# damlobster/DotsBoxesAZ

Hardware: AMD Instinct MI355X
Metric: mcts_node_expansions_per_sec (higher is better)
Workload: dtype f32 via f16x3 (hi,lo)-split MFMA, f32 accumulate; max |dp|,|dv| vs torch fp32 = 1e-6 (tests/test_hip_nn.py)

## Files before the change

dotsboxesaz_amd/build.py:

```python
import hashlib
import os
import subprocess
import sys
from concurrent.futures import ThreadPoolExecutor

HERE = os.path.dirname(os.path.abspath(__file__))
CSRC = os.path.join(HERE, "csrc")
LIB = os.path.join(HERE, "libdbaz_hip.so")
HIPCC = os.environ.get("HIPCC", "/opt/rocm/bin/hipcc")
ARCH = "gfx950"

UNITS = [
    ("tree.hip", ["-ffp-contract=off"]),
    ("engine.hip", []),
    ("nn.hip", []),
    ("replay.hip", ["-ffp-contract=off"]),
    ("train.hip", []),
    ("train_net.hip", []),
]
COMMON = ["--offload-arch=" + ARCH, "-O3", "-fPIC", "-std=c++17", "-Wall", "-Wno-unused-function"]


def source_files():
    fs = [os.path.join(CSRC, f) for f in sorted(os.listdir(CSRC)) if f.endswith((".hip", ".h"))]
    return fs + [os.path.join(os.path.dirname(HERE), "include", "dbaz.h")]


def source_hash(only=None):
    h = hashlib.sha256()
    for f in source_files():
        if only is not None and os.path.basename(f) not in only:
            continue
        h.update(os.path.basename(f).encode() + b"\0")
        h.update(open(f, "rb").read())
    return h.hexdigest()[:16]


NN_SOURCES = ("nn.hip", "nn.h", "common.h")


def _newer(target, deps):
    if not os.path.exists(target):
        return True
    t = os.path.getmtime(target)
    return any(os.path.getmtime(d) > t for d in deps)


def build(force=False, verbose=False):
    hdrs = [os.path.join(CSRC, f) for f in os.listdir(CSRC) if f.endswith(".h")]
    hdrs.append(os.path.join(os.path.dirname(HERE), "include", "dbaz.h"))
    objs, jobs = [], []
    for src, extra in UNITS:
        s = os.path.join(CSRC, src)
        o = os.path.join(CSRC, src.replace(".hip", ".o"))
        objs.append(o)
        if force or _newer(o, [s] + hdrs):
            jobs.append([HIPCC] + COMMON + extra + ["-c", s, "-o", o])

    def run(cmd):
        if verbose:
            print(" ".join(cmd), flush=True)
        r = subprocess.run(cmd, stdout=subprocess.PIPE, stderr=subprocess.STDOUT, text=True)
        if r.returncode != 0:
            raise RuntimeError("hipcc failed:\n%s\n%s" % (" ".join(cmd), r.stdout))
        return r.stdout

    sh = source_hash() + " nn=" + source_hash(NN_SOURCES)
    bo, bh = os.path.join(CSRC, "buildinfo.o"), os.path.join(CSRC, "buildinfo.hash")
    objs.append(bo)
    if force or not os.path.exists(bo) or not os.path.exists(bh) or open(bh).read() != sh:
        jobs.append(["g++", "-O1", "-fPIC", "-c", os.path.join(CSRC, "buildinfo.cpp"), "-o", bo, '-DDBAZ_SRC_HASH="%s"' % sh])

    with ThreadPoolExecutor(max_workers=4) as ex:
        outs = list(ex.map(run, jobs))
    open(bh, "w").write(sh)
    if verbose:
        for o in outs:
            if o.strip():
                print(o)
    if jobs or force or _newer(LIB, objs):
        run([HIPCC, "--offload-arch=" + ARCH, "-shared", "-fPIC", "-o", LIB] + objs)
    return LIB


if __name__ == "__main__":
    print(build(force="--force" in sys.argv, verbose=True))
```

dotsboxesaz_amd/csrc/nn.hip:

```cpp
#include <math.h>
#include <stddef.h>
#include <stdlib.h>
#include <string.h>

#include <map>
#include <string>
#include <vector>

#include "nn.h"

typedef float f32x4 __attribute__((ext_vector_type(4)));

#define CONV_THREADS 512
#define MAXT 13
#define MAXROWS 256

struct NNState {
    Geo g;
    int max_batch = 0, precision = 0;
    int kind = 0, C = 0 , Craw = 0 , blocks = 0, hc = 0, vf = 0;
    bool ready = false;
    std::map<std::string, std::vector<float>> sd;
    std::vector<float> osc_host;
    std::vector<void *> allocs;
    float *in_s = nullptr, *in_t = nullptr;
    float *w0 = nullptr, *b0 = nullptr;
    float *tw = nullptr, *tb = nullptr;
    float *tosc = nullptr;
    unsigned long long *stamp_out = nullptr;
    int *overflow = nullptr;
    int *ovf_flags = nullptr;
    float *tw32 = nullptr, *tb32 = nullptr;
    float *hw = nullptr, *hb = nullptr;
    float *w0p = nullptr;
    float osc0 = 1.0f;
    float *hwp = nullptr;
    float hosc = 1.0f;
    float *wfc = nullptr, *bfc = nullptr;
    int KP = 0, ntp = 0, ntv = 0;
    float *wv1 = nullptr, *bv1 = nullptr;
    float *hact = nullptr;
    size_t fc_lds = 0;
    float *sn_s0 = nullptr, *sn_t0 = nullptr, *sn_ts = nullptr, *sn_tt = nullptr;
    float *sn_flat = nullptr, *sn_h1 = nullptr;
    float *sn_w0 = nullptr, *sn_b0 = nullptr, *sn_ps0 = nullptr, *sn_pt0 = nullptr;
    float *sn_w1 = nullptr, *sn_b1 = nullptr, *sn_ps1 = nullptr, *sn_pt1 = nullptr;
    size_t sn_lds = 0;
    int S = 1, NT = 1, NTT = 7;
    int S_small = 0, S_mid = 0, S_big = 0, cus = 256;
    size_t conv_lds = 0;
    int c2 = 0, S_c2 = 0, NT_c2 = 0;
    int use_rem = 0;
    size_t conv_lds_c2 = 0;
};

template <int C, int NTT>
__device__ __forceinline__ void conv_lds_f32(const f32x4 *__restrict__ src4, f32x4 *dst4, const float *__restrict__ wpk,
                                             const float *__restrict__ bias, const int *vm, int rowbase, int zbase,
                                             int W, int R, int wave, int lane, int residual, int tbase,
                                             const float *post_s = nullptr, const float *post_t = nullptr)
{
    constexpr int S4 = (C + 8) / 4;
    constexpr int KC = C / 16;
    const int jrow = lane & 15, gq = lane >> 4;
    for (int ct = wave & 3; ct < C / 16; ct += 4) {
        f32x4 acc[NTT];
#pragma unroll
        for (int t = 0; t < NTT; t++) acc[t] = (f32x4){0.f, 0.f, 0.f, 0.f};
        const f32x4 *wbase = reinterpret_cast<const f32x4 *>(wpk) + (size_t)ct * 9 * KC * 64 + lane;
        int addr[NTT];
#pragma unroll
        for (int t = 0; t < NTT; t++) addr[t] = (vm[t] & 1) ? rowbase + (-W - 1) * S4 : zbase + ((rowbase + (-W - 1) * S4) & 15) - t * 16 * S4;
        f32x4 a_cur = wbase[0];
        f32x4 b_cur[NTT];
#pragma unroll
        for (int t = 0; t < NTT; t++) b_cur[t] = src4[addr[t] + t * 16 * S4];
#pragma unroll 1
        for (int tap = 0; tap < 9; tap++) {
#pragma unroll
            for (int kc = 0; kc < KC; kc++) {
                f32x4 a_nxt, b_nxt[NTT];
                if (kc == KC - 1) {
                    const int tn = tap + 1;
                    const int off = ((tn / 3 - 1) * W + (tn % 3 - 1)) * S4;
#pragma unroll
                    for (int t = 0; t < NTT; t++) addr[t] = ((vm[t] >> tn) & 1) ? rowbase + off : zbase + ((rowbase + off) & 15) - t * 16 * S4;
                    a_nxt = wbase[(size_t)(tn < 9 ? tn * KC : 0) * 64];
#pragma unroll
                    for (int t = 0; t < NTT; t++) b_nxt[t] = src4[addr[t] + t * 16 * S4];
                } else {
// ... 211 lines not shown
            }
        }
        float vmax = 0.0f;
#pragma unroll
        for (int t = 0; t < NTT; t++) {
            const int row = (tbase + t) * 16 + jrow;
            f32x4 v = acc[t] * oscale + bv;
            if (residual) {
                if constexpr (RR) {
                    v += res[t];
                } else {
                    union { unsigned int u; f16x2 h; } c0, c1, d0, d1;
                    c0.u = rh[t][0]; c1.u = rh[t][1]; d0.u = rl[t][0]; d1.u = rl[t][1];
                    v[0] += (float)c0.h[0] + (float)d0.h[0];
                    v[1] += (float)c0.h[1] + (float)d0.h[1];
                    v[2] += (float)c1.h[0] + (float)d1.h[0];
                    v[3] += (float)c1.h[1] + (float)d1.h[1];
                }
            }
            v = relu4(v);
            if constexpr (RR) {
                if (residual) res[t] = v;
            }
            if (post_s) {
                v = v * *reinterpret_cast<const f32x4 *>(post_s + ct * 16 + gq * 4) +
                    *reinterpret_cast<const f32x4 *>(post_t + ct * 16 + gq * 4);
                vmax = fmaxf(vmax, fmaxf(fmaxf(fabsf(v[0]), fabsf(v[1])), fmaxf(fabsf(v[2]), fabsf(v[3]))));
            } else {
                vmax = fmaxf(vmax, max4(v));
            }
            h3_store<C>(dsth + (size_t)row * (S4 * 8) + ct * 16 + gq * 4, row < R, v);
        }
        ovf |= vmax > F16_GUARD;
        STAMP(t3);
#ifdef DBAZ_STAMP
        if (stamps) { stamps[0] += t1 - t0; stamps[1] += t2 - t1; stamps[2] += t3 - t2; }
#endif
    }
    ovf_out |= ovf;
}

#define WRING_UNITS 512

__device__ __forceinline__ void glds16(const void *gsrc, unsigned lds_dst)
{
    unsigned keep;
    asm volatile("s_mov_b32 %0, m0\n\ts_mov_b32 m0, %2\n\ts_nop 0\n\tglobal_load_lds_dwordx4 %1, off\n\ts_mov_b32 m0, %0"
                 : "=&s"(keep) : "v"(gsrc), "s"(lds_dst) : "memory");
}
__device__ __forceinline__ unsigned lds_addr(const void *p)
{
    return (unsigned)(size_t)(const __attribute__((address_space(3))) char *)p;
}
template <int C, int NTT>
__device__ __forceinline__ void conv_lds_h3_c2(const f32x4 *__restrict__ src4, f32x4 *dst4, const f32x4 *__restrict__ wpk ,
                                               const float *__restrict__ bias, float oscale, const int *vm, int rowbase,
                                               int zbase, int W, int R, int wave, int lane, int residual, bool &ovf_out, int tbase,
                                               WPre (&pre)[2], const f32x4 *next_wpk, f32x4 (&res)[2][NTT],
                                               unsigned long long *stamps, f32x4 *wring)
{
    unsigned long long t0 = 0, t1 = 0, t2 = 0, t3 = 0;
    (void)t0; (void)t1; (void)t2; (void)t3; (void)stamps;
    static_assert(C == 64, "two cout tiles per wave x two wave parities = 64 channels");
    constexpr int S4 = (C + 8) / 4;
    constexpr int KS = C / 32;
    constexpr int LO = C / 8;
    constexpr int N = 9 * KS;
    static_assert(N % 2 == 0, "the next layer's step 0 must land in slot 0");
    const int jrow = lane & 15, gq = lane >> 4;
    const int ct0 = (wave & 1) * 2;
    f32x4 acc[2][NTT];
#pragma unroll
    for (int c = 0; c < 2; c++)
#pragma unroll
        for (int t = 0; t < NTT; t++) acc[c][t] = (f32x4){0.f, 0.f, 0.f, 0.f};
    u128h a_h[2][2], a_l[2][2];
    u128h bh[NTT], bl[NTT];
    const char *sb = reinterpret_cast<const char *>(src4);
    int ab[NTT];
    auto tap_unit = [&](int offr) -> int { return rowbase + offr * S4; };
    {
        const int u0 = tap_unit(-W - 1);
#pragma unroll
        for (int t = 0; t < NTT; t++) ab[t] = ((vm[t] & 1) ? u0 : zbase + (u0 & 15) - t * 16 * S4) * 16;
    }
    STAMP(t0);
    const f32x4 *dsrc = wpk + ((size_t)(wave >> 1) * N * 2 + (wave & 1)) * 64 + lane;
    const f32x4 *dnext = next_wpk ? next_wpk + ((size_t)(wave >> 1) * N * 2 + (wave & 1)) * 64 + lane : nullptr;
    const f32x4 *rsrc = wring + (size_t)ct0 * 2 * 64 + lane;
    const unsigned ring_dst = __builtin_amdgcn_readfirstlane(lds_addr(wring + (size_t)wave * 64));
#pragma unroll
    for (int c = 0; c < 2; c++) { a_h[c][0].f = pre[c].h0; a_l[c][0].f = pre[c].l0; }
#pragma unroll
    for (int t = 0; t < NTT; t++) bh[t].f = *reinterpret_cast<const f32x4 *>(sb + ab[t] + t * 256 * S4);
#pragma unroll
    for (int t = 0; t < NTT; t++) bl[t].f = *reinterpret_cast<const f32x4 *>(sb + ab[t] + t * 256 * S4 + LO * 16);
    STAMP(t1);
#pragma unroll
    for (int i = 0; i < N; i++) {
        const int cur = i & 1, nxt = (i + 1) & 1;
        const int ni = i + 1, ntap = ni / KS, nks = ni % KS;
        if (i + 2 < N) glds16(dsrc + (size_t)(i + 2) * 128, ring_dst + (i & 1) * (WRING_UNITS * 16));
        else if (dnext) glds16(dnext + (size_t)(i + 2 - N) * 128, ring_dst + (i & 1) * (WRING_UNITS * 16));
        if (ni < N) {
            const f32x4 *r1 = rsrc + (size_t)(ni & 1) * WRING_UNITS;
            a_h[0][nxt].f = r1[0]; a_l[0][nxt].f = r1[64]; a_h[1][nxt].f = r1[128]; a_l[1][nxt].f = r1[192];
        }
        __builtin_amdgcn_sched_barrier(0);
#pragma unroll
        for (int t = 0; t < NTT; t++) {
            acc[0][t] = __builtin_amdgcn_mfma_f32_16x16x32_f16(a_h[0][cur].h, bh[t].h, acc[0][t], 0, 0, 0);
            acc[1][t] = __builtin_amdgcn_mfma_f32_16x16x32_f16(a_h[1][cur].h, bh[t].h, acc[1][t], 0, 0, 0);
        }
        if (ni < N && nks == 0) {
            const int un = tap_unit((ntap / 3 - 1) * W + (ntap % 3 - 1));
            const int zt = zbase + (un & 15);
#pragma unroll
            for (int t = 0; t < NTT; t++) ab[t] = (((vm[t] >> ntap) & 1) ? un : zt - t * 16 * S4) * 16;
        }
        __builtin_amdgcn_sched_barrier(0);
#pragma unroll
        for (int t = 0; t < NTT; t++) {
            acc[0][t] = __builtin_amdgcn_mfma_f32_16x16x32_f16(a_l[0][cur].h, bh[t].h, acc[0][t], 0, 0, 0);
            acc[1][t] = __builtin_amdgcn_mfma_f32_16x16x32_f16(a_l[1][cur].h, bh[t].h, acc[1][t], 0, 0, 0);
            if (ni < N) bh[t].f = *reinterpret_cast<const f32x4 *>(sb + ab[t] + t * 256 * S4 + nks * 64);
            __builtin_amdgcn_sched_barrier(0);
        }
#pragma unroll
        for (int t = 0; t < NTT; t++) {
            acc[0][t] = __builtin_amdgcn_mfma_f32_16x16x32_f16(a_h[0][cur].h, bl[t].h, acc[0][t], 0, 0, 0);
            acc[1][t] = __builtin_amdgcn_mfma_f32_16x16x32_f16(a_h[1][cur].h, bl[t].h, acc[1][t], 0, 0, 0);
            if (ni < N) bl[t].f = *reinterpret_cast<const f32x4 *>(sb + ab[t] + t * 256 * S4 + nks * 64 + LO * 16);
            __builtin_amdgcn_sched_barrier(0);
        }
        if (ni < N) asm volatile("s_waitcnt vmcnt(0) lgkmcnt(%0)" ::"n"(2 * NTT) : "memory");
        else asm volatile("s_waitcnt vmcnt(0)" ::: "memory");
        if (ni < N) __builtin_amdgcn_s_barrier();
        __builtin_amdgcn_sched_barrier(0);
    }
    STAMP(t2);
    f32x4 bv[2];
#pragma unroll
    for (int c = 0; c < 2; c++) {
        bv[c] = *reinterpret_cast<const f32x4 *>(bias + (ct0 + c) * 16 + gq * 4);
        asm volatile("" ::"v"(bv[c]));
    }
    __builtin_amdgcn_sched_barrier(0);
    if (next_wpk) {
        pre[0].h0 = rsrc[0]; pre[0].l0 = rsrc[64]; pre[1].h0 = rsrc[128]; pre[1].l0 = rsrc[192];
    }
    __builtin_amdgcn_sched_barrier(0);
    _Float16 *dsth = reinterpret_cast<_Float16 *>(dst4);
    float vmax = 0.0f;
#pragma unroll
    for (int c = 0; c < 2; c++) {
        const int col = (ct0 + c) * 16 + gq * 4;
#pragma unroll
        for (int t = 0; t < NTT; t++) {
            const int row = (tbase + t) * 16 + jrow;
            f32x4 v = acc[c][t] * oscale + bv[c];
            if (residual) v += res[c][t];
            v = relu4(v);
            if (residual) res[c][t] = v;
            vmax = fmaxf(vmax, max4(v));
            h3_store<C>(dsth + (size_t)row * (S4 * 8) + col, row < R, v);
        }
    }
    ovf_out |= vmax > F16_GUARD;
    STAMP(t3);
#ifdef DBAZ_STAMP
    if (stamps) { stamps[0] += t1 - t0; stamps[1] += t2 - t1; stamps[2] += t3 - t2; }
#endif
}

__device__ __forceinline__ int cut_n(int n, int round, int defer_max)
{
    if (round <= 0) return n;
    const int n_full = (n / round) * round;
    return (n_full > 0 && n - n_full <= defer_max) ? n_full : n;
}

struct TowerArgs {
    const float *feat;
    const int32_t *list;
    const int32_t *n_dev;
    const float *in_s, *in_t;
    const float *w0, *b0;
    const float *tw;
    const float *tb;
    const float *tosc;
    const float *hw, *hb;
    const float *hwp;
    float hosc;
    const float *w0p;
    float osc0;
    unsigned long long *stamp_out;
    const float *wfc, *bfc;
    const float *wv1, *bv1;
    float *P, *V;
    int KP, ntp, ntv, vf, AS;
    int32_t *n_used;
    int *overflow;
    int *ovf_flags;
    int fallback;
    int S, nblocks, hc;
    int role, S_main, S_small, S_mid, S_big, S_huge, cus;
    int cut_round, cut_defer;
};
static_assert(offsetof(TowerArgs, wfc) == 136, "see stamp_out: the fields from wfc on keep these kernel-argument offsets");

__device__ __forceinline__ void head_fc_fused(const Geo &g, const TowerArgs &a, const float *stage, float *lg, int ns, int s0,
                                              int tid, int nthr)
{
    const int lane = tid & 63, wave = tid >> 6, nw = nthr >> 6;
    const int K = a.hc * g.HW, KC = a.KP / 16, NJ = a.ntp + a.ntv, LGS = NJ * 16 + 1, A = g.A;
    const int jrow = lane & 15, gq = lane >> 4;
    const f32x4 *wfc4 = reinterpret_cast<const f32x4 *>(a.wfc);
    const float *rowp = stage + (size_t)min(jrow, ns - 1) * (2 * K) + gq * 4;
    constexpr int G = 8;
    for (int job = wave; job < NJ; job += nw) {
        const float *brow = rowp + (job < a.ntp ? 0 : K);
        const f32x4 *wp = wfc4 + (size_t)job * KC * 64 + lane;
        f32x4 acc = (f32x4){0.f, 0.f, 0.f, 0.f};
        f32x4 wc[G], wn[G];
#pragma unroll
        for (int j = 0; j < G; j++) wc[j] = j < KC ? wp[(size_t)j * 64] : (f32x4){0.f, 0.f, 0.f, 0.f};
        for (int base = 0; base < KC; base += G) {
#pragma unroll
            for (int j = 0; j < G; j++) wn[j] = base + G + j < KC ? wp[(size_t)(base + G + j) * 64] : (f32x4){0.f, 0.f, 0.f, 0.f};
#pragma unroll
            for (int j = 0; j < G; j++)
                if (base + j < KC) {
                    const f32x4 b = *reinterpret_cast<const f32x4 *>(brow + (base + j) * 16);
#pragma unroll
                    for (int e = 0; e < 4; e++) acc = __builtin_amdgcn_mfma_f32_16x16x4f32(wc[j][e], b[e], acc, 0, 0, 0);
                }
#pragma unroll
            for (int j = 0; j < G; j++) wc[j] = wn[j];
        }
        if (jrow < ns) {
#pragma unroll
            for (int e = 0; e < 4; e++) lg[jrow * LGS + job * 16 + gq * 4 + e] = acc[e] + a.bfc[job * 16 + gq * 4 + e];
        }
    }
    __syncthreads();
    for (int sidx = wave; sidx < ns; sidx += nw) {
        const int dst = a.list ? a.list[s0 + sidx] : s0 + sidx;
        const float *l = lg + sidx * LGS;
        float mx = -INFINITY;
        for (int o = lane; o < A; o += 64) mx = fmaxf(mx, l[o]);
        for (int sh = 32; sh > 0; sh >>= 1) mx = fmaxf(mx, __shfl_xor(mx, sh));
        float sum = 0.0f;
        for (int o = lane; o < A; o += 64) sum += expf(l[o] - mx);
        for (int sh = 32; sh > 0; sh >>= 1) sum += __shfl_xor(sum, sh);
        for (int o = lane; o < A; o += 64) a.P[(size_t)dst * a.AS + o] = expf(l[o] - mx) / sum;
        float hv = 0.0f;
        for (int u = lane; u < a.vf; u += 64) hv += fmaxf(l[a.ntp * 16 + u], 0.0f) * a.wv1[u];
        for (int sh = 32; sh > 0; sh >>= 1) hv += __shfl_xor(hv, sh);
        if (lane == 0) a.V[dst] = tanhf(hv + a.bv1[0]);
    }
// ... 85 lines not shown
                    al.f = wp[64];
                    const f32x4 bv = *reinterpret_cast<const f32x4 *>(a.b0 + cto * 16 + gg * 4) * ACT_SCALE;
                    _Float16 *dsth = reinterpret_cast<_Float16 *>(X4);
                    float vmax = 0.0f;
                    for (int t = half; t < NT; t += nhalf) {
                        const int row = t * 16 + jr;
                        const int rr = min(row, R - 1);
                        u128h bh, bl;
                        bh.f = M4[(size_t)rr * MU + gg];
                        bl.f = M4[(size_t)rr * MU + 4 + gg];
                        f32x4 acc = (f32x4){0.f, 0.f, 0.f, 0.f};
                        acc = __builtin_amdgcn_mfma_f32_16x16x32_f16(ah.h, bh.h, acc, 0, 0, 0);
                        acc = __builtin_amdgcn_mfma_f32_16x16x32_f16(al.h, bh.h, acc, 0, 0, 0);
                        acc = __builtin_amdgcn_mfma_f32_16x16x32_f16(ah.h, bl.h, acc, 0, 0, 0);
                        f32x4 v = acc * a.osc0 + bv;
                        v = relu4(v);
                        vmax = fmaxf(vmax, max4(v));
                        h3_store<C>(dsth + (size_t)row * (S4 * 8) + cto * 16 + gg * 4, row < R, v);
                    }
                    ovf |= vmax > F16_GUARD;
                }
            }
        }
        if (!mfma0) {
        for (int i = tid; i < R * (C / 16); i += NTHR) {
            const int row = i % R, cq = i / R;
            const float *pp = pad + rowbase_s[row];
            float in27[27];
#pragma unroll
            for (int tap = 0; tap < 9; tap++)
#pragma unroll
                for (int c = 0; c < 3; c++) in27[tap * 3 + c] = pp[(c * PH + tap / 3) * PW + tap % 3];
#pragma unroll
            for (int q = 0; q < 4; q++) {
                const int co = cq * 16 + q * 4;
                f32x4 acc = *reinterpret_cast<const f32x4 *>(a.b0 + co);
#pragma unroll
                for (int k = 0; k < 27; k++) acc += in27[k] * *reinterpret_cast<const f32x4 *>(wl + k * C + co);
#pragma unroll
                for (int e = 0; e < 4; e++) act_store<C, PREC>(X, row, co + e, fmaxf(acc[e], 0.0f), ovf);
            }
        }
        }
        __syncthreads();
        if (tid < 3 * S4) {
            X4[zu + tid] = (f32x4){0.f, 0.f, 0.f, 0.f};
            Y4[zu + tid] = (f32x4){0.f, 0.f, 0.f, 0.f};
        }
    }
    __syncthreads();
    const int jrow = lane & 15, gq = lane >> 4;
    const bool first = wave < 4;
    const int tbase = C2 ? (wave >> 1) * NTA : (first ? 0 : NTA);
    int vm[NTA];
#pragma unroll
    for (int t = 0; t < NTA; t++) {
        int row = (tbase + t) * 16 + jrow;
        int pos = row % HW, y = pos / W, x = pos - y * W;
        int m = 0;
#pragma unroll
        for (int tap = 0; tap < 9; tap++) {
            int yy = y + tap / 3 - 1, xx = x + tap % 3 - 1;
            m |= ((yy >= 0) && (yy < H) && (xx >= 0) && (xx < W)) ? (1 << tap) : 0;
        }
        vm[t] = row < R ? m : 0;
    }
    const int rowbase = (tbase * 16 + jrow) * S4 + gq;
    const int zbase = zu;
    if constexpr (PREC == 0) {
        const size_t wl = (size_t)C * C * 9;
        for (int l = 0; l < 2 * a.nblocks; l++) {
            const f32x4 *src = (l & 1) ? Y4 : X4;
            f32x4 *dst = (l & 1) ? X4 : Y4;
            if (first) conv_lds_f32<C, NTA>(src, dst, a.tw + (size_t)l * wl, a.tb + l * C, vm, rowbase, zbase, W, R, wave, lane, l & 1, tbase);
            else if constexpr (NTB > 0) conv_lds_f32<C, NTB>(src, dst, a.tw + (size_t)l * wl, a.tb + l * C, vm, rowbase, zbase, W, R, wave, lane, l & 1, tbase);
            __syncthreads();
        }
    } else {
        const f32x4 *tw4 = reinterpret_cast<const f32x4 *>(a.tw);
        const size_t wl = (size_t)C * C * 9 * 2 * 2 / 16;
        const int NL = 2 * a.nblocks;
        WPre pre;
        WPre pre2[2];
        (void)pre2;
        if constexpr (!C2) {
            if (NL > 0) wpre_load<C>(pre, tw4, wave, lane);
        }
        unsigned long long stamps[4] = {0, 0, 0, 0};
        unsigned long long tb0 = 0, tb1 = 0, tk0 = 0, tk1 = 0;
        (void)tb0; (void)tb1; (void)tk0; (void)tk1;
        f32x4 res[2][NTA];
        (void)res;
        if constexpr (RR || C2) {
            const _Float16 *xh = reinterpret_cast<const _Float16 *>(X4);
#pragma unroll
            for (int c = 0; c < (C2 ? 2 : 1); c++) {
                const int col = (C2 ? (wave & 1) * 2 + c : wave & 3) * 16 + gq * 4;
                if (col < C) {
#pragma unroll
                    for (int t = 0; t < NTA; t++) {
                        const int row = min((tbase + t) * 16 + jrow, R - 1);
                        const _Float16 *ph = xh + (size_t)row * (S4 * 8) + col;
#pragma unroll
                        for (int e = 0; e < 4; e++) res[c][t][e] = (float)ph[e] + (float)ph[C + e];
                    }
                }
            }
        }
        f32x4 *wring = nullptr;
        if constexpr (C2) {
            wring = Y4 + img_units;
            if (NL > 0) {
                const f32x4 *d0 = tw4 + ((size_t)(wave >> 1) * (9 * (C / 32)) * 2 + (wave & 1)) * 64 + lane;
                const unsigned dst = __builtin_amdgcn_readfirstlane(lds_addr(wring + (size_t)wave * 64));
                glds16(d0, dst);
                glds16(d0 + 128, dst + WRING_UNITS * 16);
                asm volatile("s_waitcnt vmcnt(0)" ::: "memory");
            }
            __syncthreads();
            {
                const f32x4 *r0 = wring + (size_t)((wave & 1) * 2) * 2 * 64 + lane;
                pre2[0].h0 = r0[0]; pre2[0].l0 = r0[64]; pre2[1].h0 = r0[128]; pre2[1].l0 = r0[192];
                asm volatile("s_waitcnt lgkmcnt(0)" ::: "memory");
            }
            __syncthreads();
        }
        STAMP(tk0);
        tL0 = tk0;
        for (int l = 0; l < NL; l++) {
            const f32x4 *src = (l & 1) ? Y4 : X4;
            f32x4 *dst = (l & 1) ? X4 : Y4;
            const f32x4 *nxt = l + 1 < NL ? tw4 + (size_t)(l + 1) * wl : nullptr;
            if constexpr (C2) {
                conv_lds_h3_c2<C, NTA>(src, dst, tw4 + (size_t)l * wl, a.tb + l * C, a.tosc[l], vm, rowbase, zbase, W, R, wave, lane, l & 1, ovf, tbase, pre2, nxt, res, stamps, wring);
            } else {
                if (first) conv_lds_h3<C, NTA, RR>(src, dst, tw4 + (size_t)l * wl, a.tb + l * C, a.tosc[l], vm, rowbase, zbase, W, R, wave, lane, l & 1, ovf, tbase, nullptr, nullptr, pre, nxt, res[0], stamps);
                else if constexpr (NTB > 0) conv_lds_h3<C, NTB, RR>(src, dst, tw4 + (size_t)l * wl, a.tb + l * C, a.tosc[l], vm, rowbase, zbase, W, R, wave, lane, l & 1, ovf, tbase, nullptr, nullptr, pre, nxt, reinterpret_cast<f32x4(&)[NTB]>(res[0]), stamps);
            }
            STAMP(tb0);
            __syncthreads();
            STAMP(tb1);
#ifdef DBAZ_STAMP
            stamps[3] += tb1 - tb0;
#endif
        }
#ifdef DBAZ_STAMP
        STAMP(tk1);
        tL1 = tk1;
        if (a.stamp_out && lane == 0) {
            unsigned long long *o = a.stamp_out + ((size_t)blockIdx.x * 8 + wave) * 10;
            o[0] = stamps[0]; o[1] = stamps[1]; o[2] = stamps[2]; o[3] = stamps[3]; o[4] = tk1 - tk0;
        }
#endif
    }
    bool heads_done = false;
    if constexpr (PREC == 1) {
        if (a.hwp) {
            constexpr int KS = C / 32, LO = C / 8;
            const int OC = 2 * a.hc, n_ct = ((OC + 15) & ~15) / 16, ngrp = (NTHR >> 6) / n_ct;
            const int ct = wave % n_ct, grp = wave / n_ct;
            const int NT = (R + 15) / 16;
            float *stage = Y;
            const f32x4 *wp = reinterpret_cast<const f32x4 *>(a.hwp) + (size_t)ct * KS * 2 * 64 + lane;
            u128h ah[KS], al[KS];
#pragma unroll
            for (int ks = 0; ks < KS; ks++) { ah[ks].f = wp[(size_t)ks * 128]; al[ks].f = wp[(size_t)ks * 128 + 64]; }
            const int hj = lane & 15, hq = lane >> 4;
            const int oc0 = ct * 16 + hq * 4;
            f32x4 bv = (f32x4){0.f, 0.f, 0.f, 0.f};
#pragma unroll
            for (int r = 0; r < 4; r++) if (oc0 + r < OC) bv[r] = a.hb[oc0 + r];
            for (int t = grp; t < NT; t += ngrp) {
                const int row = t * 16 + hj;
                const int rr = min(row, R - 1);
                const f32x4 *bp = X4 + (size_t)rr * S4 + hq;
                f32x4 acc = (f32x4){0.f, 0.f, 0.f, 0.f};
#pragma unroll
                for (int ks = 0; ks < KS; ks++) {
                    u128h bh, bl;
                    bh.f = bp[ks * 4];
                    bl.f = bp[ks * 4 + LO];
                    acc = __builtin_amdgcn_mfma_f32_16x16x32_f16(ah[ks].h, bh.h, acc, 0, 0, 0);
                    acc = __builtin_amdgcn_mfma_f32_16x16x32_f16(al[ks].h, bh.h, acc, 0, 0, 0);
                    acc = __builtin_amdgcn_mfma_f32_16x16x32_f16(ah[ks].h, bl.h, acc, 0, 0, 0);
                }
                if (row < R) {
// ... 898 lines not shown
            if (o < ntp * 16) return o < A ? wp->data() + (size_t)o * K : nullptr;
            return o - ntp * 16 < vf ? w0->data() + (size_t)(o - ntp * 16) * K : nullptr;
        }));
        nn->bfc = nn_upload(nn, bias);
        nn->wv1 = nn_upload(nn, *w1);
        nn->bv1 = nn_upload(nn, *b1);
        nn->KP = KP; nn->ntp = ntp; nn->ntv = ntv;
    }
    if (!nn->wfc || !nn->wv1 || !nn->w0) { err = "hipMalloc failed (network buffers)"; return DBAZ_EDEVICE; }
    const size_t lds_budget = 158 * 1024;
    auto lds_bytes = [&](int S_) {
        const size_t s4 = (C + 8) / 4;
        const size_t img = ((((size_t)S_ * HW * s4 + 15) & ~(size_t)15) + 3 * s4) * 4;
        const size_t need0 = (size_t)S_ * 3 * (g.H + 2) * (g.W + 2) + (size_t)27 * C;
        const size_t nj = (size_t)(A + 15) / 16 + (size_t)(vf + 15) / 16;
        const size_t need1 = (size_t)2 * hc * (C + 4) + (size_t)S_ * 2 * hc * HW + 16 + (size_t)S_ * (nj * 16 + 1);
        return (img + std::max(img, std::max(need0, need1))) * 4;
    };
    int S = (16 * MAXT) / HW;
    if (S < 1) S = 1;
    while (S > 1 && lds_bytes(S) > lds_budget) S--;
    if (lds_bytes(S) > lds_budget) { err = "board / channels / head_channels too large for the LDS-resident tower"; return DBAZ_EINVAL; }
    nn->S = S;
    nn->NT = (S * HW + 15) / 16;
    nn->conv_lds = lds_bytes(S);
    nn->NTT = nn->NT > 8 ? 7 : (nn->NT > 4 ? 4 : 2);
    nn->S_small = nn->S_mid = nn->S_big = 0;
    if (nn->NTT == 7) {
        nn->S_big = std::min(160 / HW, nn->S - 1);
        nn->S_mid = std::max(0, std::min(128 / HW, nn->S_big - 1));
        nn->S_small = std::max(0, std::min(64 / HW, nn->S_mid - 1));
    } else if (nn->NTT == 4) {
        nn->S_small = std::min(64 / HW, nn->S - 1);
    }
    {
        int dev = 0, cus = 0;
        if (hipGetDevice(&dev) == hipSuccess && hipDeviceGetAttribute(&cus, hipDeviceAttributeMultiprocessorCount, dev) == hipSuccess && cus > 0)
            nn->cus = cus;
    }
    if (nn->c2 && C == 64) {
        int Sc = MAXROWS / HW;
        if (Sc > 16) Sc = 16;
        const size_t ring = (size_t)2 * WRING_UNITS * 16, budget_c2 = (size_t)160 * 1024 - 1536;
        while (Sc > 1 && lds_bytes(Sc) + ring > budget_c2) Sc--;
        nn->S_c2 = Sc;
        nn->NT_c2 = ((Sc * HW + 15) / 16 + 3) / 4;
        nn->conv_lds_c2 = lds_bytes(Sc) + ring;
        const double fill_c2 = (double)Sc * HW / (64.0 * nn->NT_c2), fill_1 = (double)nn->S * HW / (16.0 * nn->NT);
        if (fill_c2 < 0.9 * fill_1) nn->c2 = 0;
        if (nn->NT_c2 < 1 || nn->NT_c2 > 4 || lds_bytes(Sc) + ring > budget_c2) nn->c2 = 0;
    } else {
        nn->c2 = 0;
    }
    hipError_t he = tower_dispatch(nn, nullptr, TowerArgs(), nn->NTT, 0, true);
    nn->use_rem = (nn->precision == 1 && nn->NTT == 7 && C >= 32) ? 1 : 0;
    if (!nn->use_rem) nn->c2 = 0;
    if (he == hipSuccess && nn->use_rem) he = tower_dispatch_rem(nn, nullptr, TowerArgs(), 0, true);
    if (he == hipSuccess && nn->c2) he = tower_dispatch_c2(nn, nullptr, TowerArgs(), nn->NT_c2, 0, true);
    if (he == hipSuccess && nn->tw32) he = tower_dispatch(nn, nullptr, TowerArgs(), nn->NTT, 0, true, 0);
    if (he == hipSuccess && nn->S_mid > 0) he = tower_dispatch(nn, nullptr, TowerArgs(), 4, 0, true);
    if (he == hipSuccess && nn->S_small > 0) he = tower_dispatch(nn, nullptr, TowerArgs(), 2, 0, true);
    if (he == hipSuccess && nn->S_big > 0) he = tower_dispatch(nn, nullptr, TowerArgs(), 5, 0, true);
    if (he != hipSuccess) { err = std::string("hipFuncSetAttribute: ") + hipGetErrorString(he); return DBAZ_EDEVICE; }
    nn->ready = true;
    return DBAZ_OK;
}

void nn_forward(NNState *nn, hipStream_t s, const float *feat, const int32_t *list_dev, const int32_t *n_dev, int max_n,
                float *P, float *V, int AS, hipEvent_t ev_begin, hipEvent_t ev_end, int cut_round, int cut_defer, int32_t *n_used)
{
    const Geo &g = nn->g;
    const int hc = nn->hc;
    if (max_n > nn->max_batch) max_n = nn->max_batch;
    if (nn->kind == DBAZ_EVAL_SIMPLENN) {
        SimpleArgs sa;
        sa.feat = feat; sa.list = list_dev; sa.n_dev = n_dev; sa.w0 = nn->w0; sa.b0 = nn->b0; sa.s0 = nn->sn_s0; sa.t0 = nn->sn_t0;
        sa.tw = nn->tw; sa.tb = nn->tb; sa.ts = nn->sn_ts; sa.tt = nn->sn_tt; sa.tosc = nn->tosc; sa.flat = nn->sn_flat;
        sa.overflow = nn->overflow; sa.S = nn->S;
        if (ev_begin) (void)hipEventRecord(ev_begin, s);
        const int grid = (max_n + nn->S - 1) / nn->S;
        if (nn->precision == 1) hipLaunchKernelGGL(k_simple_trunk<1>, dim3(grid), dim3(CONV_THREADS), nn->sn_lds, s, g, sa);
        else hipLaunchKernelGGL(k_simple_trunk<0>, dim3(grid), dim3(CONV_THREADS), nn->sn_lds, s, g, sa);
        if (ev_end) (void)hipEventRecord(ev_end, s);
        DenseArgs d0;
        d0.n_dev = n_dev; d0.in = nn->sn_flat; d0.w = nn->sn_w0; d0.b = nn->sn_b0; d0.ps = nn->sn_ps0; d0.pt = nn->sn_pt0;
        d0.out = nn->sn_h1; d0.K = 1024; d0.O = 512; d0.RS4 = dense_rs4(1024); d0.dup = 0;
        hipLaunchKernelGGL(k_dense, dim3((max_n + 15) / 16), dim3(256), (size_t)16 * d0.RS4 * 16, s, d0);
        DenseArgs d1;
        d1.n_dev = n_dev; d1.in = nn->sn_h1; d1.w = nn->sn_w1; d1.b = nn->sn_b1; d1.ps = nn->sn_ps1; d1.pt = nn->sn_pt1;
        d1.out = nn->hact; d1.K = 512; d1.O = 256; d1.RS4 = dense_rs4(512); d1.dup = 1;
        hipLaunchKernelGGL(k_dense, dim3((max_n + 15) / 16), dim3(256), (size_t)16 * d1.RS4 * 16, s, d1);
        HeadArgs ha;
        ha.list = list_dev; ha.n_dev = n_dev; ha.hact = nn->hact; ha.wfc = nn->wfc; ha.bfc = nn->bfc;
        ha.P = P; ha.V = V; ha.K = 256; ha.KP = 256; ha.ntp = nn->ntp; ha.ntv = nn->ntv; ha.AS = AS;
        hipLaunchKernelGGL(k_head_fc, dim3((max_n + 16 * HEAD_MT - 1) / (16 * HEAD_MT)), dim3(256), nn->fc_lds, s, g, ha);
        return;
    }
    TowerArgs ta;
    ta.feat = feat; ta.list = list_dev; ta.n_dev = n_dev; ta.in_s = nn->in_s; ta.in_t = nn->in_t; ta.w0 = nn->w0; ta.b0 = nn->b0;
    ta.tw = nn->tw; ta.tb = nn->tb; ta.tosc = nn->tosc; ta.hw = nn->hw; ta.hb = nn->hb; ta.hwp = nn->hwp; ta.hosc = nn->hosc; ta.w0p = nn->w0p; ta.osc0 = nn->osc0;
    ta.overflow = nn->overflow; ta.ovf_flags = nn->ovf_flags; ta.fallback = 0; ta.S = nn->S; ta.nblocks = nn->blocks; ta.hc = hc;
    ta.wfc = nn->wfc; ta.bfc = nn->bfc; ta.wv1 = nn->wv1; ta.bv1 = nn->bv1; ta.P = P; ta.V = V; ta.KP = nn->KP; ta.ntp = nn->ntp;
    ta.ntv = nn->ntv; ta.vf = nn->vf; ta.AS = AS; ta.n_used = n_used;
    ta.stamp_out = nn->stamp_out;
    if (ev_begin) (void)hipEventRecord(ev_begin, s);
    ta.S_main = nn->S; ta.S_small = nn->S_small; ta.S_mid = nn->S_mid; ta.S_big = nn->S_big; ta.S_huge = 0; ta.cus = nn->cus;
    ta.cut_round = cut_round; ta.cut_defer = cut_defer;
    ta.role = 0; ta.S = nn->S;
    if (nn->c2) {
        ta.S_main = ta.S = nn->S_c2; ta.S_huge = nn->S;
        (void)tower_dispatch_c2(nn, s, ta, nn->NT_c2, (max_n + nn->S_c2 - 1) / nn->S_c2, false);
    }
    if (!nn->c2) (void)tower_dispatch(nn, s, ta, nn->NTT, (max_n + nn->S - 1) / nn->S, false);
    if (nn->use_rem) {
        ta.role = -1;
        (void)tower_dispatch_rem(nn, s, ta, nn->cus, false);
    } else {
        if (nn->S_small > 0) {
            ta.role = 1; ta.S = nn->S_small;
            (void)tower_dispatch(nn, s, ta, 2, nn->cus, false);
        }
        if (nn->S_mid > 0) {
            ta.role = 2; ta.S = nn->S_mid;
            (void)tower_dispatch(nn, s, ta, 4, nn->cus, false);
        }
        if (nn->S_big > 0) {
            ta.role = 3; ta.S = nn->S_big;
            (void)tower_dispatch(nn, s, ta, 5, nn->cus, false);
        }
    }
    if (nn->precision == 1 && nn->tw32) {
        ta.role = 0; ta.S = ta.S_main = nn->S; ta.S_small = ta.S_mid = ta.S_big = ta.S_huge = 0; ta.fallback = 1;
        ta.tw = nn->tw32; ta.tb = nn->tb32; ta.w0p = nullptr; ta.hwp = nullptr;
        (void)tower_dispatch(nn, s, ta, nn->NTT, std::min((max_n + nn->S - 1) / nn->S, nn->cus), false, 0);
    }
    if (ev_end) (void)hipEventRecord(ev_end, s);
}

void nn_round_info(const NNState *nn, int *round, int *rem_max)
{
    *round = 0; *rem_max = 0;
    if (!nn || nn->kind != DBAZ_EVAL_RESNET) return;
    *round = nn->cus * (nn->c2 ? nn->S_c2 : nn->S);
    const int s_rem = nn->c2 ? nn->S : std::max(nn->S_big, std::max(nn->S_mid, nn->S_small));
    *rem_max = nn->cus * s_rem;
}

double nn_flops_per_sample(const NNState *nn)
{
    const Geo &g = nn->g;
    if (nn->kind == DBAZ_EVAL_SIMPLENN)
        return 2.0 * (16 * 27 * 256 + 3.0 * 16 * 2304 * 256 + 4 * 2304 * 256 + 1024 * 512 + 512 * 256 + 256 * 33);
    const double HW = g.HW, C = nn->Craw, hc = nn->hc, K = hc * HW;
    double f = 2.0 * HW * 27 * C + 2.0 * nn->blocks * 2.0 * HW * 9 * C * C;
    f += 2.0 * 2.0 * HW * C * hc + 2.0 * K * g.A + 2.0 * K * nn->vf + 2.0 * nn->vf;
    return f;
}

int nn_read_stamps(NNState *nn, unsigned long long *out, int n_wg)
{
    if (!nn || !nn->stamp_out) return -1;
// ... 19 lines not shown
```

Before: 4.655 million.

## Permute tower rows so edge tiles skip out-of-board conv taps

Adds a host-built row permutation table that groups board positions into 16-row tiles sharing a missing edge (top, bottom, left, right). Each wave pair is assigned one edge pattern, and the conv kernel is specialised per pattern at compile time so the MFMAs and LDS loads for always-zero taps are skipped. Outputs are stored back through the permuted row index. This cuts MFMA work on boundary tiles, at the cost of gathered addressing, a switch over template instances (code size), and waitcnt counts that vary per tap.

New measurement: 4.756 million (median of 6 runs). +2.2%, better.

```diff
diff --git a/dotsboxesaz_amd/build.py b/dotsboxesaz_amd/build.py
--- a/dotsboxesaz_amd/build.py
+++ b/dotsboxesaz_amd/build.py
@@ -36,7 +36,7 @@
     return h.hexdigest()[:16]
 
 
-NN_SOURCES = ("nn.hip", "nn.h", "common.h")
+NN_SOURCES = ("nn.hip", "nn.h", "common.h", "tower_perm.h")
 
 
 def _newer(target, deps):
diff --git a/dotsboxesaz_amd/csrc/nn.hip b/dotsboxesaz_amd/csrc/nn.hip
--- a/dotsboxesaz_amd/csrc/nn.hip
+++ b/dotsboxesaz_amd/csrc/nn.hip
@@ -8,6 +8,7 @@
 #include <vector>
 
 #include "nn.h"
+#include "tower_perm.h"
 
 typedef float f32x4 __attribute__((ext_vector_type(4)));
 
@@ -36,6 +37,7 @@
     float osc0 = 1.0f;
     float *hwp = nullptr;
     float hosc = 1.0f;
+    unsigned char *tperm = nullptr;
     float *wfc = nullptr, *bfc = nullptr;
     int KP = 0, ntp = 0, ntv = 0;
     float *wv1 = nullptr, *bv1 = nullptr;
@@ -353,13 +355,27 @@
 {
     return (unsigned)(size_t)(const __attribute__((address_space(3))) char *)p;
 }
-template <int C, int NTT>
+#define PAT_NONE 4
+__host__ __device__ constexpr int pat_drop(int pat, int t)
+{
+    constexpr int top = 0007, bottom = 0700, left = 0111, right = 0444;
+    return pat == PAT_NONE || t > 1 ? 0
+         : t == 0 ? (pat < 2 ? top : bottom)
+                  : (pat == 0 || pat == 3 ? left : right);
+}
+static_assert(pat_drop(0, 0) == TP_TOP && pat_drop(0, 1) == TP_LEFT && pat_drop(1, 0) == TP_TOP && pat_drop(1, 1) == TP_RIGHT &&
+              pat_drop(2, 0) == TP_BOTTOM && pat_drop(2, 1) == TP_RIGHT && pat_drop(3, 0) == TP_BOTTOM && pat_drop(3, 1) == TP_LEFT,
+              "the kernel's patterns are those the row table is built and verified for (tower_perm.h)");
+
+template <int C, int NTT, int PAT = PAT_NONE>
 __device__ __forceinline__ void conv_lds_h3_c2(const f32x4 *__restrict__ src4, f32x4 *dst4, const f32x4 *__restrict__ wpk ,
                                                const float *__restrict__ bias, float oscale, const int *vm, int rowbase,
                                                int zbase, int W, int R, int wave, int lane, int residual, bool &ovf_out, int tbase,
                                                WPre (&pre)[2], const f32x4 *next_wpk, f32x4 (&res)[2][NTT],
-                                               unsigned long long *stamps, f32x4 *wring)
-{
+                                               unsigned long long *stamps, f32x4 *wring, const int *rb = nullptr)
+{
+    constexpr bool PERM = PAT != PAT_NONE;
+    static_assert(!PERM || NTT == 4, "the row table is built for 4 tiles per wave pair");
     unsigned long long t0 = 0, t1 = 0, t2 = 0, t3 = 0;
     (void)t0; (void)t1; (void)t2; (void)t3; (void)stamps;
     static_assert(C == 64, "two cout tiles per wave x two wave parities = 64 channels");
@@ -380,11 +396,27 @@
     const char *sb = reinterpret_cast<const char *>(src4);
     int ab[NTT];
     auto tap_unit = [&](int offr) -> int { return rowbase + offr * S4; };
-    {
-        const int u0 = tap_unit(-W - 1);
-#pragma unroll
-        for (int t = 0; t < NTT; t++) ab[t] = ((vm[t] & 1) ? u0 : zbase + (u0 & 15) - t * 16 * S4) * 16;
-    }
+    auto kept = [](int t, int tap) constexpr -> bool { return !((pat_drop(PAT, t) >> tap) & 1); };
+    auto n_kept = [&](int tap) constexpr -> int { int n = 0; for (int t = 0; t < NTT; t++) n += kept(t, tap) ? 1 : 0; return n; };
+    auto tile_off = [](int t) constexpr -> int { return PERM ? 0 : t * 256 * S4; };
+    auto set_ab = [&](int tap) {
+        if constexpr (PERM) {
+            int offu = ((tap / 3 - 1) * W + (tap % 3 - 1)) * S4;
+            asm volatile("" : "+s"(offu));
+#pragma unroll
+            for (int t = 0; t < NTT; t++)
+                if (kept(t, tap)) {
+                    const int un = rb[t] + offu;
+                    ab[t] = (((vm[t] >> tap) & 1) ? un : zbase + (un & 15)) * 16;
+                }
+        } else {
+            const int un = tap_unit((tap / 3 - 1) * W + (tap % 3 - 1));
+            const int zt = zbase + (un & 15);
+#pragma unroll
+            for (int t = 0; t < NTT; t++) ab[t] = (((vm[t] >> tap) & 1) ? un : zt - t * 16 * S4) * 16;
+        }
+    };
+    set_ab(0);
     STAMP(t0);
     const f32x4 *dsrc = wpk + ((size_t)(wave >> 1) * N * 2 + (wave & 1)) * 64 + lane;
     const f32x4 *dnext = next_wpk ? next_wpk + ((size_t)(wave >> 1) * N * 2 + (wave & 1)) * 64 + lane : nullptr;
@@ -393,14 +425,16 @@
 #pragma unroll
     for (int c = 0; c < 2; c++) { a_h[c][0].f = pre[c].h0; a_l[c][0].f = pre[c].l0; }
 #pragma unroll
-    for (int t = 0; t < NTT; t++) bh[t].f = *reinterpret_cast<const f32x4 *>(sb + ab[t] + t * 256 * S4);
-#pragma unroll
-    for (int t = 0; t < NTT; t++) bl[t].f = *reinterpret_cast<const f32x4 *>(sb + ab[t] + t * 256 * S4 + LO * 16);
+    for (int t = 0; t < NTT; t++)
+        if (kept(t, 0)) bh[t].f = *reinterpret_cast<const f32x4 *>(sb + ab[t] + tile_off(t));
+#pragma unroll
+    for (int t = 0; t < NTT; t++)
+        if (kept(t, 0)) bl[t].f = *reinterpret_cast<const f32x4 *>(sb + ab[t] + tile_off(t) + LO * 16);
     STAMP(t1);
 #pragma unroll
     for (int i = 0; i < N; i++) {
         const int cur = i & 1, nxt = (i + 1) & 1;
-        const int ni = i + 1, ntap = ni / KS, nks = ni % KS;
+        const int tap = i / KS, ni = i + 1, ntap = ni / KS, nks = ni % KS;
         if (i + 2 < N) glds16(dsrc + (size_t)(i + 2) * 128, ring_dst + (i & 1) * (WRING_UNITS * 16));
         else if (dnext) glds16(dnext + (size_t)(i + 2 - N) * 128, ring_dst + (i & 1) * (WRING_UNITS * 16));
         if (ni < N) {
@@ -409,33 +443,36 @@
         }
         __builtin_amdgcn_sched_barrier(0);
 #pragma unroll
+        for (int t = 0; t < NTT; t++)
+            if (kept(t, tap)) {
+                acc[0][t] = __builtin_amdgcn_mfma_f32_16x16x32_f16(a_h[0][cur].h, bh[t].h, acc[0][t], 0, 0, 0);
+                acc[1][t] = __builtin_amdgcn_mfma_f32_16x16x32_f16(a_h[1][cur].h, bh[t].h, acc[1][t], 0, 0, 0);
+            }
+        if (ni < N && nks == 0) set_ab(ntap);
+        __builtin_amdgcn_sched_barrier(0);
+#pragma unroll
         for (int t = 0; t < NTT; t++) {
-            acc[0][t] = __builtin_amdgcn_mfma_f32_16x16x32_f16(a_h[0][cur].h, bh[t].h, acc[0][t], 0, 0, 0);
-            acc[1][t] = __builtin_amdgcn_mfma_f32_16x16x32_f16(a_h[1][cur].h, bh[t].h, acc[1][t], 0, 0, 0);
-        }
-        if (ni < N && nks == 0) {
-            const int un = tap_unit((ntap / 3 - 1) * W + (ntap % 3 - 1));
-            const int zt = zbase + (un & 15);
-#pragma unroll
-            for (int t = 0; t < NTT; t++) ab[t] = (((vm[t] >> ntap) & 1) ? un : zt - t * 16 * S4) * 16;
-        }
-        __builtin_amdgcn_sched_barrier(0);
+            if (kept(t, tap)) {
+                acc[0][t] = __builtin_amdgcn_mfma_f32_16x16x32_f16(a_l[0][cur].h, bh[t].h, acc[0][t], 0, 0, 0);
+                acc[1][t] = __builtin_amdgcn_mfma_f32_16x16x32_f16(a_l[1][cur].h, bh[t].h, acc[1][t], 0, 0, 0);
+            }
+            if (ni < N && kept(t, ntap)) bh[t].f = *reinterpret_cast<const f32x4 *>(sb + ab[t] + tile_off(t) + nks * 64);
+            __builtin_amdgcn_sched_barrier(0);
+        }
 #pragma unroll
         for (int t = 0; t < NTT; t++) {
-            acc[0][t] = __builtin_amdgcn_mfma_f32_16x16x32_f16(a_l[0][cur].h, bh[t].h, acc[0][t], 0, 0, 0);
-            acc[1][t] = __builtin_amdgcn_mfma_f32_16x16x32_f16(a_l[1][cur].h, bh[t].h, acc[1][t], 0, 0, 0);
-            if (ni < N) bh[t].f = *reinterpret_cast<const f32x4 *>(sb + ab[t] + t * 256 * S4 + nks * 64);
+            if (kept(t, tap)) {
+                acc[0][t] = __builtin_amdgcn_mfma_f32_16x16x32_f16(a_h[0][cur].h, bl[t].h, acc[0][t], 0, 0, 0);
+                acc[1][t] = __builtin_amdgcn_mfma_f32_16x16x32_f16(a_h[1][cur].h, bl[t].h, acc[1][t], 0, 0, 0);
+            }
+            if (ni < N && kept(t, ntap)) bl[t].f = *reinterpret_cast<const f32x4 *>(sb + ab[t] + tile_off(t) + nks * 64 + LO * 16);
             __builtin_amdgcn_sched_barrier(0);
         }
-#pragma unroll
-        for (int t = 0; t < NTT; t++) {
-            acc[0][t] = __builtin_amdgcn_mfma_f32_16x16x32_f16(a_h[0][cur].h, bl[t].h, acc[0][t], 0, 0, 0);
-            acc[1][t] = __builtin_amdgcn_mfma_f32_16x16x32_f16(a_h[1][cur].h, bl[t].h, acc[1][t], 0, 0, 0);
-            if (ni < N) bl[t].f = *reinterpret_cast<const f32x4 *>(sb + ab[t] + t * 256 * S4 + nks * 64 + LO * 16);
-            __builtin_amdgcn_sched_barrier(0);
-        }
-        if (ni < N) asm volatile("s_waitcnt vmcnt(0) lgkmcnt(%0)" ::"n"(2 * NTT) : "memory");
-        else asm volatile("s_waitcnt vmcnt(0)" ::: "memory");
+        if (ni >= N) asm volatile("s_waitcnt vmcnt(0)" ::: "memory");
+        else if (n_kept(ntap) == NTT) asm volatile("s_waitcnt vmcnt(0) lgkmcnt(%0)" ::"n"(2 * NTT) : "memory");
+        else if (n_kept(ntap) == NTT - 1) asm volatile("s_waitcnt vmcnt(0) lgkmcnt(%0)" ::"n"(2 * NTT - 2) : "memory");
+        else if (n_kept(ntap) == NTT - 2) asm volatile("s_waitcnt vmcnt(0) lgkmcnt(%0)" ::"n"(2 * NTT > 4 ? 2 * NTT - 4 : 0) : "memory");
+        else asm volatile("s_waitcnt vmcnt(0) lgkmcnt(0)" ::: "memory");
         if (ni < N) __builtin_amdgcn_s_barrier();
         __builtin_amdgcn_sched_barrier(0);
     }
@@ -458,13 +495,17 @@
         const int col = (ct0 + c) * 16 + gq * 4;
 #pragma unroll
         for (int t = 0; t < NTT; t++) {
-            const int row = (tbase + t) * 16 + jrow;
             f32x4 v = acc[c][t] * oscale + bv[c];
             if (residual) v += res[c][t];
             v = relu4(v);
             if (residual) res[c][t] = v;
             vmax = fmaxf(vmax, max4(v));
-            h3_store<C>(dsth + (size_t)row * (S4 * 8) + col, row < R, v);
+            if constexpr (PERM) {
+                h3_store<C>(dsth + (rb[t] - gq) * 8 + col, vm[t] != 0, v);
+            } else {
+                const int row = (tbase + t) * 16 + jrow;
+                h3_store<C>(dsth + (size_t)row * (S4 * 8) + col, row < R, v);
+            }
         }
     }
     ovf_out |= vmax > F16_GUARD;
@@ -507,6 +548,7 @@
     int S, nblocks, hc;
     int role, S_main, S_small, S_mid, S_big, S_huge, cus;
     int cut_round, cut_defer;
+    const unsigned char *perm;
 };
 static_assert(offsetof(TowerArgs, wfc) == 136, "see stamp_out: the fields from wfc on keep these kernel-argument offsets");
 
@@ -698,10 +740,21 @@
     const int jrow = lane & 15, gq = lane >> 4;
     const bool first = wave < 4;
     const int tbase = C2 ? (wave >> 1) * NTA : (first ? 0 : NTA);
+    constexpr bool PERMOK = C2 && NTA == 4;
+    bool perm_on = false;
+    if constexpr (PERMOK) perm_on = a.perm != nullptr;
     int vm[NTA];
+    int rb[NTA];
+    int rrow[NTA];
+    (void)rb; (void)rrow;
 #pragma unroll
     for (int t = 0; t < NTA; t++) {
         int row = (tbase + t) * 16 + jrow;
+        if constexpr (PERMOK) {
+            if (perm_on) row = a.perm[row];
+            rb[t] = row * S4 + gq;
+            rrow[t] = min(row, R - 1);
+        }
         int pos = row % HW, y = pos / W, x = pos - y * W;
         int m = 0;
 #pragma unroll
@@ -745,7 +798,8 @@
                 if (col < C) {
 #pragma unroll
                     for (int t = 0; t < NTA; t++) {
-                        const int row = min((tbase + t) * 16 + jrow, R - 1);
+                        int row = min((tbase + t) * 16 + jrow, R - 1);
+                        if constexpr (PERMOK) row = rrow[t];
                         const _Float16 *ph = xh + (size_t)row * (S4 * 8) + col;
 #pragma unroll
                         for (int e = 0; e < 4; e++) res[c][t][e] = (float)ph[e] + (float)ph[C + e];
@@ -773,11 +827,23 @@
         }
         STAMP(tk0);
         tL0 = tk0;
+        const int pat = perm_on ? __builtin_amdgcn_readfirstlane(wave >> 1) : PAT_NONE;
+        (void)pat;
         for (int l = 0; l < NL; l++) {
             const f32x4 *src = (l & 1) ? Y4 : X4;
             f32x4 *dst = (l & 1) ? X4 : Y4;
             const f32x4 *nxt = l + 1 < NL ? tw4 + (size_t)(l + 1) * wl : nullptr;
-            if constexpr (C2) {
+            if constexpr (PERMOK) {
+#define C2_PAT(P) conv_lds_h3_c2<C, NTA, P>(src, dst, tw4 + (size_t)l * wl, a.tb + l * C, a.tosc[l], vm, rowbase, zbase, W, R, wave, lane, l & 1, ovf, tbase, pre2, nxt, res, stamps, wring, rb)
+                switch (pat) {
+                case 0: C2_PAT(0); break;
+                case 1: C2_PAT(1); break;
+                case 2: C2_PAT(2); break;
+                case 3: C2_PAT(3); break;
+                default: C2_PAT(PAT_NONE); break;
+                }
+#undef C2_PAT
+            } else if constexpr (C2) {
                 conv_lds_h3_c2<C, NTA>(src, dst, tw4 + (size_t)l * wl, a.tb + l * C, a.tosc[l], vm, rowbase, zbase, W, R, wave, lane, l & 1, ovf, tbase, pre2, nxt, res, stamps, wring);
             } else {
                 if (first) conv_lds_h3<C, NTA, RR>(src, dst, tw4 + (size_t)l * wl, a.tb + l * C, a.tosc[l], vm, rowbase, zbase, W, R, wave, lane, l & 1, ovf, tbase, nullptr, nullptr, pre, nxt, res[0], stamps);
@@ -1782,6 +1848,14 @@
     } else {
         nn->c2 = 0;
     }
+    nn->tperm = nullptr;
+    if (nn->c2 && nn->NT_c2 == 4) {
+        int tab[TOWER_PERM_ROWS];
+        if (tower_perm_build(g.H, g.W, nn->S_c2, tab) > 0) {
+            nn->tperm = nn_upload(nn, std::vector<unsigned char>(tab, tab + TOWER_PERM_ROWS));
+            if (!nn->tperm) { err = "hipMalloc failed (row table)"; return DBAZ_EDEVICE; }
+        }
+    }
     hipError_t he = tower_dispatch(nn, nullptr, TowerArgs(), nn->NTT, 0, true);
     nn->use_rem = (nn->precision == 1 && nn->NTT == 7 && C >= 32) ? 1 : 0;
     if (!nn->use_rem) nn->c2 = 0;
@@ -1837,6 +1911,7 @@
     ta.S_main = nn->S; ta.S_small = nn->S_small; ta.S_mid = nn->S_mid; ta.S_big = nn->S_big; ta.S_huge = 0; ta.cus = nn->cus;
     ta.cut_round = cut_round; ta.cut_defer = cut_defer;
     ta.role = 0; ta.S = nn->S;
+    ta.perm = nn->c2 ? nn->tperm : nullptr;
     if (nn->c2) {
         ta.S_main = ta.S = nn->S_c2; ta.S_huge = nn->S;
         (void)tower_dispatch_c2(nn, s, ta, nn->NT_c2, (max_n + nn->S_c2 - 1) / nn->S_c2, false);
diff --git a/dotsboxesaz_amd/csrc/tower_perm.h b/dotsboxesaz_amd/csrc/tower_perm.h
--- /dev/null
+++ b/dotsboxesaz_amd/csrc/tower_perm.h
@@ -0,0 +1,101 @@
+#pragma once
+
+#define TOWER_PERM_ROWS 256
+#define TOWER_PERM_TILES 16
+
+enum { TP_TOP = 0007, TP_BOTTOM = 0700, TP_LEFT = 0111, TP_RIGHT = 0444 };
+
+static inline int tower_perm_drop(int T)
+{
+    static const int edge[4][2] = {{TP_TOP, TP_LEFT}, {TP_TOP, TP_RIGHT}, {TP_BOTTOM, TP_RIGHT}, {TP_BOTTOM, TP_LEFT}};
+    return (T & 3) < 2 ? edge[T >> 2][T & 3] : 0;
+}
+
+static inline int tower_perm_inside(int H, int W, int y, int x)
+{
+    int m = 0;
+    for (int tap = 0; tap < 9; tap++) {
+        const int yy = y + tap / 3 - 1, xx = x + tap % 3 - 1;
+        if (yy >= 0 && yy < H && xx >= 0 && xx < W) m |= 1 << tap;
+    }
+    return m;
+}
+
+static inline int tower_perm_build(int H, int W, int S, int *tab)
+{
+    enum { NR = TOWER_PERM_ROWS, NTL = TOWER_PERM_TILES };
+    for (int i = 0; i < NR; i++) tab[i] = i;
+    if (H < 1 || W < 1 || S < 1) return 0;
+    const int HW = H * W, R = S * HW;
+    if (R > NR || ((R + 15) / 16 + 3) / 4 != 4) return 0;
+    const int cls_mask[4] = {TP_TOP, TP_BOTTOM, TP_LEFT, TP_RIGHT};
+    int caps[NR], owner[NR];
+    int have[5] = {0, 0, 0, 0, 0};
+    for (int r = 0; r < NR; r++) {
+        caps[r] = 15;
+        if (r < R) {
+            const int p = r % HW, in = tower_perm_inside(H, W, p / W, p % W);
+            caps[r] = 0;
+            for (int k = 0; k < 4; k++)
+                if (!(in & cls_mask[k])) caps[r] |= 1 << k;
+        }
+        owner[r] = 4;
+    }
+    for (int pass = 0; pass < 3; pass++)
+        for (int r = 0; r < NR; r++) {
+            if (owner[r] != 4 || caps[r] == 0) continue;
+            const bool single = (caps[r] & (caps[r] - 1)) == 0;
+            if (pass == 0 ? !single : pass == 1 ? (single || r >= R) : r < R) continue;
+            int best = -1;
+            for (int k = 0; k < 4; k++)
+                if ((caps[r] >> k & 1) && have[k] < 32 && (best < 0 || have[k] < have[best])) best = k;
+            if (best >= 0) { owner[r] = best; have[best]++; }
+        }
+    for (int k = 0; k < 4; k++)
+        if (have[k] != 32) return 0;
+    static const int cls_tiles[5][8] = {{0, 4}, {8, 12}, {1, 13}, {5, 9}, {2, 3, 6, 7, 10, 11, 14, 15}};
+    static const int lane_set[2][8] = {{4, 5, 6, 7, 8, 9, 10, 11}, {0, 1, 2, 3, 12, 13, 14, 15}};
+    bool used[NR];
+    for (int r = 0; r < NR; r++) used[r] = false;
+    for (int k = 0; k < 5; k++) {
+        const int ntl = k < 4 ? 2 : 8;
+        for (int ti = 0; ti < ntl; ti++)
+            for (int h = 0; h < 2; h++) {
+                bool res_used[8] = {false, false, false, false, false, false, false, false};
+                for (int q = 0; q < 8; q++) {
+                    int left[8] = {0, 0, 0, 0, 0, 0, 0, 0};
+                    for (int r = 0; r < NR; r++)
+                        if (owner[r] == k && !used[r]) left[r & 7]++;
+                    int br = -1;
+                    for (int m = 0; m < 8; m++)
+                        if (left[m] > 0 && !res_used[m] && (br < 0 || left[m] > left[br])) br = m;
+                    if (br < 0)
+                        for (int m = 0; m < 8; m++)
+                            if (left[m] > 0 && (br < 0 || left[m] > left[br])) br = m;
+                    if (br < 0) { for (int i = 0; i < NR; i++) tab[i] = i; return 0; }
+                    int r = 0;
+                    while (owner[r] != k || used[r] || (r & 7) != br) r++;
+                    used[r] = true;
+                    res_used[br] = true;
+                    tab[cls_tiles[k][ti] * 16 + lane_set[h][q]] = r;
+                }
+            }
+    }
+    int seen[NR], dropped = 0;
+    for (int r = 0; r < NR; r++) seen[r] = 0;
+    bool ok = true;
+    for (int T = 0; T < NTL; T++) {
+        const int drop = tower_perm_drop(T);
+        for (int tap = 0; tap < 9; tap++) dropped += drop >> tap & 1;
+        for (int j = 0; j < 16; j++) {
+            const int r = tab[T * 16 + j];
+            if (r < 0 || r >= NR || seen[r]++) { ok = false; continue; }
+            if (r < R && (tower_perm_inside(H, W, (r % HW) / W, (r % HW) % W) & drop)) ok = false;
+        }
+    }
+    if (!ok) {
+        for (int i = 0; i < NR; i++) tab[i] = i;
+        return 0;
+    }
+    return dropped;
+}
```
